# megvii-research/OccDepth

Measured on AMD Instinct MI355X. Metric: frames/sec forward, SemanticKITTI stereo->256x256x32 voxels, higher is better.
Workload: dtype f32 storage and accumulate; matrix arithmetic as 3x bf16 split (hi + mid + lo of both operands, six v_mfma_f32_32x32x16_bf16 per K step; error vs float64 tested within 1.5x of the exact-fp32 kernels', measured 0.8-1.1x) in the head convolutions (K2s3), the small-volume 3x3x3 convolutions and transpo

## Files before the change

### occdepth_amd/csrc/conv3d_bf16.hip

```cpp
#include "device.h"

#include <algorithm>
#include <cstddef>
#include <cstdlib>
#include <cstring>

using occd::FastDiv;

namespace {

struct PhaseBP {
    const u32x4* wpk;
    int KX, KY, KZ, oox, ooy, ooz, YIN, ZIN;
    FastDiv div_zin;
};
constexpr int kMaxPhasesB = 8;

struct ConvBP {
    const void* in;
    const float* bias;
    const void* res1;
    const void* res2;
    void* out;
    int X, Y, Z, cin8, cin16, in_cs, in_coff;
    int K16tot, NTtot;
    int out_cs, out_coff, res1_cs, res1_coff, res2_cs, res2_coff;
    int SX, SY, SZ, DX, DY, DZ, PX, PY, PZ;
    int Xo, Yo, Zo, OX, OY, OZ, osx, osy, osz;
    int act_in, act_out, cout_store;
    int TY, TZ, ytiles, ztiles, nwg;
    int nph_log2;
    int ph_fast;
    FastDiv div_tz, div_ztiles, div_ytiles;
    PhaseBP ph[kMaxPhasesB];
};

__device__ __forceinline__ f32x4 unpack_lo(u32x2 v) {
    f32x4 r;
    r.x = __builtin_bit_cast(float, v.x << 16);
    r.y = __builtin_bit_cast(float, v.x & 0xffff0000u);
    r.z = __builtin_bit_cast(float, v.y << 16);
    r.w = __builtin_bit_cast(float, v.y & 0xffff0000u);
    return r;
}

constexpr int kRSB = 80;
constexpr int kRSB3 = 208;


template <int MT, int NT, int WM, int WN, bool IN_BF16, bool OUT_BF16, int SPLIT = 1, int KS = 1>
__global__ void __launch_bounds__(WM* WN * KS * 64) conv3d_bf16_kernel(const ConvBP p) {
    constexpr int NTH = WM * WN * 64;
    constexpr int RSB = SPLIT == 3 ? kRSB3 : kRSB;
    static_assert(SPLIT == 1 || (SPLIT == 3 && !IN_BF16 && !OUT_BF16), "the 3-way split takes and returns float32");
    extern __shared__ __attribute__((aligned(16))) unsigned char slab_all[];

    const int lane = threadIdx.x & 63;
    const int wave_all = __builtin_amdgcn_readfirstlane(threadIdx.x >> 6);
    const int kg = KS == 1 ? 0 : wave_all / (WM * WN);
    const int wave = wave_all - kg * (WM * WN);
    const int tid = threadIdx.x - kg * NTH;
    const int wm = wave / WN;
    const int wn = wave - wm * WN;
    const int li = lane & 31;
    const int h = lane >> 5;

    uint32_t bid = xcd_remap(blockIdx.x, p.nwg);
    const uint32_t ph_mask = (1u << p.nph_log2) - 1u;
    const uint32_t ph_i = p.ph_fast ? bid & ph_mask : blockIdx.y & ph_mask;
    if (p.ph_fast) bid >>= p.nph_log2;
    const uint32_t t1 = occd_fastdiv(bid, p.div_ztiles);
    const int zt = bid - t1 * p.ztiles;
    const uint32_t t2 = occd_fastdiv(t1, p.div_ytiles);
    const int yt = t1 - t2 * p.ytiles;
    const int xo = t2;
    const int b = p.ph_fast ? blockIdx.y : blockIdx.y >> p.nph_log2;
    const PhaseBP& ph = p.ph[ph_i];
// ... 16 lines not shown

    f32x16 acc[MT][NT];
#pragma unroll
    for (int mt = 0; mt < MT; ++mt)
#pragma unroll
        for (int nt = 0; nt < NT; ++nt)
#pragma unroll
            for (int r = 0; r < 16; ++r) acc[mt][nt][r] = 0.f;

    const int y_in0 = yt * p.TY * p.SY - p.PY;
    const int z_in0 = zt * p.TZ * p.SZ - p.PZ;
    const size_t w_step = (size_t)p.NTtot * 64;
    const size_t w_img = (size_t)ph.KX * ph.KY * ph.KZ * p.K16tot * w_step;
    const u32x4* const wlane = ph.wpk + lane;
    const int rows = ph.YIN * ph.ZIN;
    unsigned char* const slab = slab_all + (size_t)kg * rows * RSB;
    const int n_chunks = (p.cin16 + 31) / 32;
    const int chunk_iters = (n_chunks + KS - 1) / KS;

#define OCCD_MFMA1(WS, XS)                                                                                          \
    _Pragma("unroll") for (int nt = 0; nt < NT; ++nt) _Pragma("unroll") for (int mt = 0; mt < MT; ++mt) acc[mt][nt] = \
        __builtin_amdgcn_mfma_f32_32x32x16_bf16(__builtin_bit_cast(bf16x8, b_cur[nt][WS]),                         \
                                                __builtin_bit_cast(bf16x8, a_cur[mt][XS]), acc[mt][nt], 0, 0, 0)
#define OCCD_MFMA_BLOCK()                                                  \
    if (SPLIT == 3) {                                                      \
        OCCD_MFMA1(SPLIT == 3 ? 1 : 0, SPLIT == 3 ? 1 : 0);                \
        OCCD_MFMA1(0, SPLIT == 3 ? 2 : 0);                                 \
        OCCD_MFMA1(SPLIT == 3 ? 2 : 0, 0);                                 \
        OCCD_MFMA1(0, SPLIT == 3 ? 1 : 0);                                 \
        OCCD_MFMA1(SPLIT == 3 ? 1 : 0, 0);                                 \
    }                                                                      \
    OCCD_MFMA1(0, 0)

    for (int kx = 0; kx < ph.KX; ++kx) {
        const int xi = xo * p.SX - p.PX + kx * p.DX;
        if (xi < 0 || xi >= p.X) continue;
        const size_t plane = ((size_t)(b * p.X + xi) * p.Y) * p.Z * p.in_cs + p.in_coff;
        for (int ci = 0; ci < chunk_iters; ++ci) {
            const int c0 = (ci * KS + kg) * 32;
            const bool active = KS == 1 || c0 < p.cin16;
            const int ck = active ? min(32, p.cin16 - c0) : 16;
            const int k16n = ck >> 4;
            const int sh = k16n;
            const int S = active ? ph.KY * ph.KZ * k16n : 0;
            const u32x4* wp = wlane + ((size_t)(kx * ph.KY * ph.KZ) * p.K16tot + (active ? c0 >> 4 : 0)) * w_step;

            u32x4 b_cur[NT][SPLIT];
#pragma unroll
            for (int nt = 0; nt < NT; ++nt)
#pragma unroll
                for (int sp = 0; sp < SPLIT; ++sp) b_cur[nt][sp] = wp[wofs[nt] + sp * w_img];

            __syncthreads();
            const int F = rows << sh;
            for (int f0 = 0; active && f0 < F; f0 += NTH * 4) {
                u32x4 v[4][SPLIT];
                int dst[4];
#pragma unroll
                for (int u = 0; u < 4; ++u) {
                    const int f = f0 + u * NTH + tid;
                    const int fc = min(f, F - 1);
                    const uint32_t row = (uint32_t)fc >> sh;
                    const int c8 = fc & ((1 << sh) - 1);
                    const uint32_t yi = occd_fastdiv(row, ph.div_zin);
                    const int zi = (int)row - (int)yi * ph.ZIN;
                    const int y = y_in0 + (int)yi, z = z_in0 + zi;
                    const int c = c0 + c8 * 8;
                    const bool ok = f < F && c < p.cin8 && (unsigned)y < (unsigned)p.Y && (unsigned)z < (unsigned)p.Z;
                    const int yc = min(max(y, 0), p.Y - 1), zc = min(max(z, 0), p.Z - 1);
                    const int cc = min(c, p.cin8 - 8);
                    const size_t e = plane + ((size_t)yc * p.Z + zc) * p.in_cs + cc;
                    u32x4 w[SPLIT];
                    if (IN_BF16) {
                        w[0] = *(const u32x4*)((const uint16_t*)p.in + e);
                        if (p.act_in == OCCD_ACT_RELU) {
#pragma unroll
                            for (int q = 0; q < 4; ++q) {
                                uint32_t d = w[0][q];
                                if (d & 0x80000000u) d &= 0x0000ffffu;
                                if (d & 0x00008000u) d &= 0xffff0000u;
                                w[0][q] = d;
                            }
                        }
                    } else {
                        f32x4 lo = *(const f32x4*)((const float*)p.in + e);
                        f32x4 hi = *(const f32x4*)((const float*)p.in + e + 4);
                        if (p.act_in == OCCD_ACT_RELU) { lo = act3d_x4(lo, OCCD_ACT_RELU); hi = act3d_x4(hi, OCCD_ACT_RELU); }
                        else if (SPLIT == 3 && p.act_in == OCCD_ACT_SIGMOID) {
                            lo = act3d_x4(lo, OCCD_ACT_SIGMOID); hi = act3d_x4(hi, OCCD_ACT_SIGMOID);
                        }
                        if (SPLIT == 3) split3_bf16x8(lo, hi, w[0], w[SPLIT == 3 ? 1 : 0], w[SPLIT == 3 ? 2 : 0]);
                        else w[0] = pack_bf16x8(lo, hi);
                    }
#pragma unroll
                    for (int sp = 0; sp < SPLIT; ++sp) v[u][sp] = ok ? w[sp] : u32x4{0u, 0u, 0u, 0u};
                    dst[u] = f < F ? (int)row * RSB + c8 * 16 : -1;
                }
#pragma unroll
                for (int u = 0; u < 4; ++u)
                    if (dst[u] >= 0) {
#pragma unroll
                        for (int sp = 0; sp < SPLIT; ++sp) *(u32x4*)(slab + dst[u] + sp * 64) = v[u][sp];
                    }
            }
            __syncthreads();

            int ky = 0, kz = 0, kl = 0;
            int lds_off = 0;
            u32x4 a_cur[MT][SPLIT];
#pragma unroll
            for (int mt = 0; mt < MT; ++mt)
#pragma unroll
                for (int sp = 0; sp < SPLIT; ++sp) a_cur[mt][sp] = *(const u32x4*)(slab + rowbase[mt] + sp * 64);

            for (int s = 0; s < S - 1; ++s) {
                ++kl;
                lds_off += 32;
                wp += w_step;
                if (kl == k16n) {
                    kl = 0;
                    wp += (size_t)(p.K16tot - k16n) * w_step;
                    if (++kz == ph.KZ) { kz = 0; ++ky; }
                    lds_off = (ky * p.DY * ph.ZIN + kz * p.DZ) * RSB;
                }
                u32x4 a_nxt[MT][SPLIT], b_nxt[NT][SPLIT];
#pragma unroll
                for (int mt = 0; mt < MT; ++mt)
#pragma unroll
                    for (int sp = 0; sp < SPLIT; ++sp) a_nxt[mt][sp] = *(const u32x4*)(slab + rowbase[mt] + lds_off + sp * 64);
#pragma unroll
                for (int nt = 0; nt < NT; ++nt)
#pragma unroll
                    for (int sp = 0; sp < SPLIT; ++sp) b_nxt[nt][sp] = wp[wofs[nt] + sp * w_img];
                OCCD_MFMA_BLOCK();
#pragma unroll
                for (int mt = 0; mt < MT; ++mt)
#pragma unroll
                    for (int sp = 0; sp < SPLIT; ++sp) a_cur[mt][sp] = a_nxt[mt][sp];
#pragma unroll
                for (int nt = 0; nt < NT; ++nt)
#pragma unroll
                    for (int sp = 0; sp < SPLIT; ++sp) b_cur[nt][sp] = b_nxt[nt][sp];
            }
            if (active) { OCCD_MFMA_BLOCK(); }
        }
    }
#undef OCCD_MFMA1
#undef OCCD_MFMA_BLOCK

    if (KS > 1) {
        float* red = reinterpret_cast<float*>(slab_all);
        __syncthreads();
        if (kg > 0) {
#pragma unroll
            for (int mt = 0; mt < MT; ++mt)
#pragma unroll
                for (int nt = 0; nt < NT; ++nt)
#pragma unroll
                    for (int r = 0; r < 16; ++r)
                        red[((((kg - 1) * WM * WN + wave) * MT + mt) * NT + nt) * 1024 + r * 64 + lane] = acc[mt][nt][r];
        }
        __syncthreads();
        if (kg > 0) return;
#pragma unroll
        for (int g = 1; g < KS; ++g)
#pragma unroll
            for (int mt = 0; mt < MT; ++mt)
#pragma unroll
                for (int nt = 0; nt < NT; ++nt)
#pragma unroll
                    for (int r = 0; r < 16; ++r)
                        acc[mt][nt][r] += red[((((g - 1) * WM * WN + wave) * MT + mt) * NT + nt) * 1024 + r * 64 + lane];
    }

#pragma unroll
    for (int mt = 0; mt < MT; ++mt) {
        const uint32_t m = (wm * MT + mt) * 32 + li;
        const uint32_t yl = occd_fastdiv(m, p.div_tz);
        const uint32_t zl = m - yl * p.TZ;
        const int yo = yt * p.TY + (int)yl, zo = zt * p.TZ + (int)zl;
        const bool ok = yl < (uint32_t)p.TY && yo < p.Yo && zo < p.Zo;
        const size_t vox = ((size_t)(b * p.OX + xo * p.osx + ph.oox) * p.OY + (yo * p.osy + ph.ooy)) * p.OZ +
                           (zo * p.osz + ph.ooz);
#pragma unroll
        for (int nt = 0; nt < NT; ++nt) {
#pragma unroll
            for (int g = 0; g < 4; ++g) {
                const int c = (nt0 + nt) * 32 + 8 * g + 4 * h;
                if (ok && c < p.cout_store) {
                    f32x4 v = {acc[mt][nt][4 * g], acc[mt][nt][4 * g + 1], acc[mt][nt][4 * g + 2],
                               acc[mt][nt][4 * g + 3]};
                    if (p.bias != nullptr) v += *(const f32x4*)(p.bias + c);
                    if (p.act_out == OCCD_ACT_RELU_PRE) v = act3d_x4(v, OCCD_ACT_RELU);
                    if (OUT_BF16) {
                        if (p.res1 != nullptr)
                            v += unpack_lo(*(const u32x2*)((const uint16_t*)p.res1 + vox * p.res1_cs + p.res1_coff + c));
                        if (p.res2 != nullptr)
                            v += unpack_lo(*(const u32x2*)((const uint16_t*)p.res2 + vox * p.res2_cs + p.res2_coff + c));
                    } else {
                        if (p.res1 != nullptr) v += *(const f32x4*)((const float*)p.res1 + vox * p.res1_cs + p.res1_coff + c);
                        if (p.res2 != nullptr) v += *(const f32x4*)((const float*)p.res2 + vox * p.res2_cs + p.res2_coff + c);
                    }
                    if (p.act_out == OCCD_ACT_RELU) v = act3d_x4(v, OCCD_ACT_RELU);
                    if (OUT_BF16) {
                        bf16x4 o = {(__bf16)v.x, (__bf16)v.y, (__bf16)v.z, (__bf16)v.w};
                        *(u32x2*)((uint16_t*)p.out + vox * p.out_cs + p.out_coff + c) = __builtin_bit_cast(u32x2, o);
                    } else {
                        *(f32x4*)((float*)p.out + vox * p.out_cs + p.out_coff + c) = v;
                    }
                }
            }
        }
    }
}
// ... 58 lines not shown
    const int lane = (i >> 3) & 63;
    long t = i >> 9;
    const int nt = t % NT; t /= NT;
    const int k16 = t % K16; t /= K16;
    const int tap = (int)t;
    const int co = nt * 32 + (lane & 31);
    const int ci = k16 * 16 + (lane >> 5) * 8 + j;
    float v = 0.f;
    if (co < cout && ci < cin) {
        if (layout == 0) v = w[((size_t)co * cin + ci) * taps + tap];
        else if (layout == 1) v = w[((size_t)ci * cout + co) * taps + tap];
        else v = w[(size_t)ci * cout + co];
        if (scale != nullptr) v *= scale[co];
        v *= 0.5f / fac[co];
    }
    const _Float16 hi = (_Float16)v;
    wpk[i] = __builtin_bit_cast(uint16_t, hi);
    wpk[i + total] = __builtin_bit_cast(uint16_t, (_Float16)((float)hi * (1.f / 2048.f)));
    wpk[i + 2 * total] = __builtin_bit_cast(uint16_t, (_Float16)(v - (float)hi));
}

struct VariantB {
    int MT, NT, WM, WN, KS;
    void (*kern[3])(const ConvBP);
};

#define OCCD_VARIANT_B(MT, NT, WM, WN) \
    VariantB { MT, NT, WM, WN, 1, { conv3d_bf16_kernel<MT, NT, WM, WN, false, false>, conv3d_bf16_kernel<MT, NT, WM, WN, true, true>, nullptr } }
#define OCCD_VARIANT_B3(MT, NT, WM, WN) \
    VariantB { MT, NT, WM, WN, 1, { conv3d_bf16_kernel<MT, NT, WM, WN, false, false>, conv3d_bf16_kernel<MT, NT, WM, WN, true, true>, \
                                    conv3d_bf16_kernel<MT, NT, WM, WN, false, false, 3> } }

const VariantB kVariantsB[] = {
    OCCD_VARIANT_B(4, 1, 4, 1),
    OCCD_VARIANT_B3(2, 1, 4, 1),
    OCCD_VARIANT_B3(1, 1, 4, 1),
    OCCD_VARIANT_B(4, 2, 4, 1),
    OCCD_VARIANT_B3(2, 2, 4, 1),
    OCCD_VARIANT_B(4, 2, 2, 2),
    OCCD_VARIANT_B3(2, 2, 2, 2),
    OCCD_VARIANT_B3(1, 2, 2, 2),
    VariantB { 1, 1, 1, 4, 4, { nullptr, nullptr, conv3d_bf16_kernel<1, 1, 1, 4, false, false, 3, 4> } },
};
constexpr int kNumVariantsB = sizeof(kVariantsB) / sizeof(kVariantsB[0]);
constexpr size_t kMaxLdsB = 160 * 1024;

struct TilingB {
    int TY, TZ, YIN, ZIN, ytiles, ztiles, ngroups;
    size_t lds;
    long nwg;
    double cost;
};

bool plan_b(const occd_conv3d_args* a, const VariantB& v, int NTtot, TilingB* best, int rsb) {
    const int mwg = v.MT * v.WM * 32;
    bool found = false;
    int cands[16];
    int nc = 0;
    if (a->Zo <= mwg) cands[nc++] = a->Zo;
    for (int tz = 8; tz <= mwg; tz *= 2)
        if (tz < a->Zo) cands[nc++] = tz;
    for (int i = 0; i < nc; ++i) {
        TilingB t;
        t.TZ = cands[i];
        t.TY = mwg / t.TZ;
// ... 92 lines not shown
    return pack_bf16_gather(w, scale, wpk, cout, cin, ntaps, s_co, s_ci, tap_ofs, 3, stream);
}

static int pack_bf16_gather(const float* w, const float* scale, void* wpk, int32_t cout, int32_t cin, int32_t ntaps,
                            int64_t s_co, int64_t s_ci, const int32_t* tap_ofs, int nsplit, void* stream) {
    if (!w || !wpk || !tap_ofs || ntaps <= 0 || ntaps > occd::kMaxTaps) return OCCD_EINVAL;
    const int64_t total = occd_packed_weight_bf16_elems(cout, cin, ntaps);
    if (total <= 0) return OCCD_EINVAL;
    occd::TapMap tm{};
    tm.s_co = s_co; tm.s_ci = s_ci;
    for (int i = 0; i < ntaps; ++i) tm.ofs[i] = tap_ofs[i];
    const int K16 = (cin + 15) / 16, NT = (cout + 31) / 32;
    const int th = 256;
    const long blocks = (total + th - 1) / th;
    occd::ProfScope prof("pack_weights_bf16", (hipStream_t)stream, 0.0, (double)total * 6);
    hipLaunchKernelGGL(pack_weights_bf16_kernel, dim3((unsigned)blocks), dim3(th), 0, (hipStream_t)stream, w, scale,
                       (uint16_t*)wpk, cout, cin, ntaps, K16, NT, 3, (long)total, nsplit, tm);
    return occd::check_launch();
}

namespace {

int validate_b(const occd_conv3d_args* a, int32_t dtype) {
    if (!a || !a->in || !a->wpk || !a->out || dtype < 0 || dtype > 3) return OCCD_EINVAL;
    const int ksel = dtype;
    if (dtype >= 2) dtype = 0;
    if (a->batch <= 0 || a->X <= 0 || a->Y <= 0 || a->Z <= 0 || a->cin <= 0 || a->cout <= 0) return OCCD_EINVAL;
    if (a->kx <= 0 || a->ky <= 0 || a->kz <= 0 || a->sx <= 0 || a->sy <= 0 || a->sz <= 0) return OCCD_EINVAL;
    if (a->Xo <= 0 || a->Yo <= 0 || a->Zo <= 0) return OCCD_EINVAL;
    const int cin8 = (a->cin + 7) & ~7;
    const int cin16 = (a->cin + 15) & ~15;
    const int NTtot = (a->cout + 31) / 32;
    const int al = dtype == 1 ? 7 : 3;
    const int esz = dtype == 1 ? 2 : 4;
    if ((a->in_cs & al) || (a->in_coff & al) || a->in_coff + cin8 > a->in_cs) return OCCD_EINVAL;
    if ((reinterpret_cast<uintptr_t>(a->in) & 15) || (reinterpret_cast<uintptr_t>(a->wpk) & 15)) return OCCD_EINVAL;
    if (a->cout_store < a->cout || a->cout_store > NTtot * 32 || a->out_coff + a->cout_store > a->out_cs)
        return OCCD_EINVAL;
    if ((a->cout_store & 3) || (a->out_cs & 3) || (a->out_coff & 3) ||
        (reinterpret_cast<uintptr_t>(a->out) & (4 * esz - 1)))
        return OCCD_EINVAL;
    if (a->res1 && ((a->res1_cs & 3) || (a->res1_coff & 3) || (reinterpret_cast<uintptr_t>(a->res1) & (4 * esz - 1)) ||
                    a->res1_coff + a->cout_store > a->res1_cs))
        return OCCD_EINVAL;
    if (a->res2 && ((a->res2_cs & 3) || (a->res2_coff & 3) || (reinterpret_cast<uintptr_t>(a->res2) & (4 * esz - 1)) ||
                    a->res2_coff + a->cout_store > a->res2_cs))
        return OCCD_EINVAL;
    if (a->bias && (reinterpret_cast<uintptr_t>(a->bias) & 15)) return OCCD_EINVAL;
    if ((a->Xo - 1) * a->o_stride_x + a->o_off_x >= a->OX || (a->Yo - 1) * a->o_stride_y + a->o_off_y >= a->OY ||
        (a->Zo - 1) * a->o_stride_z + a->o_off_z >= a->OZ)
        return OCCD_EINVAL;
    if (a->act_in != OCCD_ACT_NONE && a->act_in != OCCD_ACT_RELU && !(a->act_in == OCCD_ACT_SIGMOID && ksel == 2)) return OCCD_EINVAL;
    if (a->act_out != OCCD_ACT_NONE && a->act_out != OCCD_ACT_RELU && a->act_out != OCCD_ACT_RELU_PRE)
        return OCCD_EINVAL;
    return OCCD_OK;
}

int launch_b(const occd_conv3d_args* a, int n, int32_t dtype, hipStream_t stream) {
    const int ksel = dtype;
    if (dtype == 2) dtype = 0;
    const int esz = dtype == 1 ? 2 : 4;
    const int cin8 = (a->cin + 7) & ~7;
    const int cin16 = (a->cin + 15) & ~15;
    const int NTtot = (a->cout + 31) / 32;
    occd_conv3d_args big = a[0];
    for (int i = 1; i < n; ++i) {
        big.ky = a[i].ky > big.ky ? a[i].ky : big.ky;
        big.kz = a[i].kz > big.kz ? a[i].kz : big.kz;
    }
    const long copies = (long)a->batch * n;
    int order[kNumVariantsB];
    int no = 0;
    if (a->tile_hint > 0 && a->tile_hint <= kNumVariantsB) {
        order[no++] = a->tile_hint - 1;
    } else if (NTtot == 1) {
        order[no++] = 0; order[no++] = 1; order[no++] = 2;
    } else if (NTtot == 2) {
        order[no++] = 3; order[no++] = 4; order[no++] = 6; order[no++] = 7;
    } else {
        order[no++] = 5; order[no++] = 6; order[no++] = 7;
    }
    const int rsb = ksel == 2 ? kRSB3 : kRSB;
    int pick = -1;
    TilingB til{};
    for (int i = 0; i < no; ++i) {
        TilingB t{};
        if (kVariantsB[order[i]].kern[ksel] == nullptr) continue;
        if (!plan_b(&big, kVariantsB[order[i]], NTtot, &t, rsb)) continue;
        pick = order[i];
        til = t;
        if (t.nwg * t.ngroups * copies >= 512) break;
    }
    if (pick < 0) return OCCD_ENOMEM;
    if (ksel == 2 && a->tile_hint == 0 && til.nwg * til.ngroups * copies <= 320 && cin16 >= 128 && NTtot % 4 == 0) {
        TilingB t{};
        if (plan_b(&big, kVariantsB[8], NTtot, &t, rsb) && t.nwg * t.ngroups * copies <= 1024) {
            pick = 8;
            til = t;
        }
    }
    const VariantB& v = kVariantsB[pick];

    ConvBP p{};
    p.in = a->in; p.bias = a->bias; p.res1 = a->res1; p.res2 = a->res2; p.out = a->out;
    p.X = a->X; p.Y = a->Y; p.Z = a->Z; p.cin8 = cin8; p.cin16 = cin16; p.in_cs = a->in_cs; p.in_coff = a->in_coff;
    p.K16tot = cin16 / 16; p.NTtot = NTtot;
    p.out_cs = a->out_cs; p.out_coff = a->out_coff;
    p.res1_cs = a->res1_cs; p.res1_coff = a->res1_coff; p.res2_cs = a->res2_cs; p.res2_coff = a->res2_coff;
    p.SX = a->sx; p.SY = a->sy; p.SZ = a->sz;
    p.DX = a->dx; p.DY = a->dy; p.DZ = a->dz; p.PX = a->px; p.PY = a->py; p.PZ = a->pz;
    p.Xo = a->Xo; p.Yo = a->Yo; p.Zo = a->Zo; p.OX = a->OX; p.OY = a->OY; p.OZ = a->OZ;
    p.osx = a->o_stride_x; p.osy = a->o_stride_y; p.osz = a->o_stride_z;
    p.act_in = a->act_in; p.act_out = a->act_out; p.cout_store = a->cout_store;
    p.TY = til.TY; p.TZ = til.TZ;
    p.ytiles = til.ytiles; p.ztiles = til.ztiles; p.nwg = (int)til.nwg;
    p.div_tz = occd::make_fastdiv(til.TZ);
    p.div_ztiles = occd::make_fastdiv(til.ztiles); p.div_ytiles = occd::make_fastdiv(til.ytiles);
    p.nph_log2 = n == 1 ? 0 : n == 2 ? 1 : n == 4 ? 2 : 3;
    static const bool phase_fast = occd::env_flag("OCCD_PHASE_FAST", false);
    p.ph_fast = n > 1 && phase_fast ? 1 : 0;
    if (p.ph_fast) p.nwg = (int)(til.nwg * n);
    if (til.nwg * n >= (1L << 24)) return OCCD_EINVAL;
    int ord[kMaxPhasesB];
    for (int i = 0; i < n; ++i) ord[i] = i;
    std::stable_sort(ord, ord + n, [&](int l, int r) { return a[l].kx * a[l].ky * a[l].kz > a[r].kx * a[r].ky * a[r].kz; });
    double flops = 0.0, bytes = 0.0;
    const double pos = (double)a->batch * a->Xo * a->Yo * a->Zo;
    for (int i = 0; i < n; ++i) {
        const occd_conv3d_args* ai = a + ord[i];
        PhaseBP& ph = p.ph[i];
        ph.wpk = (const u32x4*)ai->wpk;
        ph.KX = ai->kx; ph.KY = ai->ky; ph.KZ = ai->kz;
        ph.oox = ai->o_off_x; ph.ooy = ai->o_off_y; ph.ooz = ai->o_off_z;
        ph.YIN = (til.TY - 1) * ai->sy + (ai->ky - 1) * ai->dy + 1;
        ph.ZIN = (til.TZ - 1) * ai->sz + (ai->kz - 1) * ai->dz + 1;
        ph.div_zin = occd::make_fastdiv(ph.ZIN);
        if ((size_t)ph.YIN * ph.ZIN * rsb * v.KS > til.lds) return OCCD_EINVAL;
        const double taps = (double)ai->kx * ai->ky * ai->kz;
        flops += 2.0 * pos * taps * ai->cin * ai->cout;
        bytes += (double)esz * ((i == 0 ? (double)a->batch * a->X * a->Y * a->Z * a->cin : 0.0) +
                                pos * a->cout * (1 + (a->res1 != nullptr) + (a->res2 != nullptr))) + 2.0 * taps * a->cin * a->cout;
    }
    if (copies > 65535) return OCCD_EINVAL;

    void (*kern)(const ConvBP) = v.kern[ksel];
    if (til.lds > 64 * 1024 && occd::ensure_big_lds(reinterpret_cast<const void*>(kern)) != OCCD_OK) return OCCD_ELAUNCH;
    occd::ProfScope prof(n > 1 ? "conv3d_bf16x3_phases" : ksel == 2 ? "conv3d_bf16x3" : dtype == 1 ? "conv3d_bf16s" : "conv3d_bf16",
                         stream, flops, bytes);
    hipLaunchKernelGGL(kern, p.ph_fast ? dim3((unsigned)(til.nwg * n), (unsigned)a->batch, (unsigned)til.ngroups)
                                       : dim3((unsigned)til.nwg, (unsigned)copies, (unsigned)til.ngroups),
                       dim3(v.WM * v.WN * v.KS * 64), til.lds, stream, p);
    return occd::check_launch();
}

}

extern "C" int occd_conv3d_bf16_fwd(const occd_conv3d_args* a, int32_t dtype, void* stream) {
    const int bad = validate_b(a, dtype);
    if (bad != OCCD_OK) return bad;
    if (dtype == 3) {
        const int r = occd::try_conv3d_c32_slide_x3(a, (hipStream_t)stream, true);
        return r < 0 ? r : r == 0 ? OCCD_EINVAL : OCCD_OK;
    }
    if (dtype == 2) {
        const int r = occd::try_conv3d_c32_slide_x3(a, (hipStream_t)stream);
        if (r != 0) return r < 0 ? r : OCCD_OK;
    }
    return launch_b(a, 1, dtype, (hipStream_t)stream);
}

// ... 13 lines not shown
```

### occdepth_amd/fused.py

```python
import os

import torch

from . import hip
from .hip import ACT_NONE, ACT_RELU, ACT_RELU_PRE, ACT_SIGMOID, Vox


_warned_eval_with_grad = False


def needs_autograd(module):
    if module.training:
        return True
    if torch.is_grad_enabled():
        global _warned_eval_with_grad
        if not _warned_eval_with_grad:
            _warned_eval_with_grad = True
            import warnings
            warnings.warn("occdepth_amd: eval-mode forward with autograd enabled runs the differentiable ATen path; "
                          "wrap inference in torch.no_grad() to take the HIP eval path", stacklevel=3)
        return True
    return False


# ... 95 lines not shown
BF16X3 = _parse_bf16x3(os.environ.get("OCCDEPTH_BF16X3", "head"))


def set_bf16x3(on):
    global BF16X3
    BF16X3 = "all" if on is True else _parse_bf16x3(str(on)) if on else False


def _parse_head_split(v):
    v = (v or "f16x2").strip().lower()
    if v not in ("f16x2", "bf16x3"):
        raise ValueError(f"OCCDEPTH_HEAD_SPLIT={v!r}: expected f16x2 or bf16x3")
    return v


HEAD_SPLIT = _parse_head_split(os.environ.get("OCCDEPTH_HEAD_SPLIT", "f16x2"))


def set_head_split(v):
    global HEAD_SPLIT
    HEAD_SPLIT = _parse_head_split(v)


class _DualW:

    def __init__(self, f32, x3, f16x2=None):
        self.f32, self.x3, self.f16x2 = f32, x3, f16x2


BF16X3_DILATED = os.environ.get("OCCDEPTH_BF16X3_DILATED", "0") == "1"


def _head_weight(w, layout):
    return layout == 0 and w.dim() == 5 and tuple(w.shape[2:]) == (3, 3, 3) and w.shape[0] <= 32 and 24 < w.shape[1] <= 32


BF16X3_SMALLVOL = os.environ.get("OCCDEPTH_BF16X3_SMALLVOL", "1") == "1"
SMALLVOL_MAX_VOXELS = 8192
SMALLVOL_KERNELS = ((3, 3, 3), (1, 1, 1)) if os.environ.get("OCCDEPTH_BF16X3_SMALLVOL_K1", "0") == "1" else ((3, 3, 3),)


def _smallvol_weight(w, layout):
    if not BF16X3_SMALLVOL:
        return False
    if layout == 2:
        return (1, 1, 1) in SMALLVOL_KERNELS and w.dim() == 2 and w.shape[0] >= 128 and w.shape[0] % 16 == 0 and w.shape[1] % 128 == 0
    return (layout == 0 and w.dim() == 5 and tuple(w.shape[2:]) in SMALLVOL_KERNELS and w.shape[1] >= 128
            and w.shape[1] % 16 == 0 and w.shape[0] % 128 == 0)


def _f16x2_ok(w, scale):
    if not w.is_cuda:
        return False
    ws = w if scale is None else w * scale.view(-1, *([1] * (w.dim() - 1)))
    return bool(torch.isfinite(ws).all())


def _pack_w(w, scale=None, layout=0):
    if BF16X3 == "all" or (BF16X3 == "head" and (_head_weight(w, layout) or _smallvol_weight(w, layout))):
        f16 = (hip.pack_weights_f16x2(w, scale, layout)
               if HEAD_SPLIT == "f16x2" and _head_weight(w, layout) and _f16x2_ok(w, scale) else None)
        return _DualW(hip.pack_weights(w, scale, layout), hip.pack_weights_bf16(w, scale, layout, split3=True), f16)
    return hip.pack_weights(w, scale, layout)


def _smallvol_eligible(x, wpk, cout, kernel, out, **kw):
    if not BF16X3_SMALLVOL or tuple(kernel) not in SMALLVOL_KERNELS or kw.get("cin") not in (None, x.C) or x.C < 128 or cout % 128:
        return False
    if x.cs % 8 or x.coff % 8 or x.buf.dtype != torch.float32:
        return False
    pos = kw.get("out_pos")
    if pos is None:
        st, dl, pd = kw.get("stride", (1, 1, 1)), kw.get("dilation", (1, 1, 1)), kw.get("padding", (0, 0, 0))
        pos = tuple((n + 2 * p - d * (k - 1) - 1) // s + 1 for n, p, d, s, k in zip(x.dims, pd, dl, st, kernel))
    return x.batch * pos[0] * pos[1] * pos[2] <= SMALLVOL_MAX_VOXELS and kw.get("tile_hint", 0) == 0


def _conv3d(x, wpk, bias, cout, kernel, out, **kw):
    if isinstance(wpk, _DualW):
        if hip.c32x3_eligible(x, cout, kernel, out, **kw):
            if wpk.f16x2 is not None:
                return hip.conv3d_f16x2(x, wpk.f16x2, bias, cout, kernel, out, **kw)
            return hip.conv3d_bf16(x, wpk.x3, bias, cout, kernel, out, split3=True, **kw)
        if _smallvol_eligible(x, wpk, cout, kernel, out, **kw):
            return hip.conv3d_bf16(x, wpk.x3, bias, cout, kernel, out, split3=True, **kw)
        aligned = x.cs % 8 == 0 and x.coff % 8 == 0
        dil = tuple(kw.get("dilation", (1, 1, 1)))
        big = kernel[0] * kernel[1] * kernel[2] >= 8
        if BF16X3 == "all" and aligned and big and (dil == (1, 1, 1) or BF16X3_DILATED) and kw.get("cin") is None and \
                kw.get("act_in", ACT_NONE) in (ACT_NONE, ACT_RELU):
            return hip.conv3d_bf16(x, wpk.x3, bias, cout, kernel, out, split3=True, **kw)
        wpk = wpk.f32
    return hip.conv3d(x, wpk, bias, cout, kernel, out, **kw)


class ConvPlan:

    def __init__(self, conv, bn=None, pool=None):
        self.conv, self.bn = conv, bn
        self.pool = _triple(pool) if pool is not None else None
        self._key = None
        self._wpk = self._bias = None

    @property
    def cout(self):
        return self.conv.out_channels

    def _prepare(self):
        key = (_stamp(self.conv, self.bn), BF16X3, HEAD_SPLIT)
        if key == self._key:
            return
        w = self.conv.weight.detach().float()
        dev = w.device
        cout = self.cout
        scale, shift = _bn_affine(self.bn, cout, dev)
        if self.conv.bias is not None:
            cb = self.conv.bias.detach().float()
            shift = shift + (cb * scale if scale is not None else cb)
        if self.pool is not None:
            kx, ky, kz = self.pool
            w = (w / float(kx * ky * kz)).expand(-1, -1, kx, ky, kz).contiguous()
        self._wpk = _pack_w(w, scale)
        self._bias = _pad_bias(shift, cout)
        self._wrows = None
        if self.pool is None and tuple(w.shape[2:]) == (1, 1, 1) and _triple(self.conv.stride) == (1, 1, 1):
            w2 = w.reshape(cout, -1)
            if ROWS_GEMM and w2.is_cuda and w2.shape[1] % 16 == 0 and cout % 8 == 0:
                self._wrows = hip.RowsGemmWeights((w2 * scale.view(-1, 1) if scale is not None else w2).t().contiguous())
        self._key = key

    def geometry(self):
        if self.pool is not None:
# ... 7 lines not shown

    def __call__(self, x, out=None, res1=None, res2=None, act_in=ACT_NONE, act_out=ACT_NONE):
        self._prepare()
        k, s, d, p = self.geometry()
        if out is None:
            out = Vox.empty(x.batch, self.out_dims(x.dims), self.cout, x.buf.device)
        if (ROWS_GEMM and self._wrows is not None and res2 is None and x.buf.is_cuda and _rows_gemm_wins(x, self._wrows.K)
                and hip.rows_gemm_supported(self._wrows.K, self.cout, x, out, res1)):
            return hip.rows_gemm(x, self._wrows, out, bias=self._bias, res=res1, act_in=act_in, act_out=act_out)
        return _conv3d(x, self._wpk, self._bias, self.cout, k, out, stride=s, dilation=d, padding=p,
                          res1=res1, res2=res2, act_in=act_in, act_out=act_out)


class DerivedConvPlan:

    def __init__(self, modules, derive, padding=(1, 1, 1), dilation=(1, 1, 1), stride=(1, 1, 1)):
        self.modules, self.derive = list(modules), derive
        self.padding, self.dilation, self.stride = padding, dilation, stride
        self._key = None
        self._wpk = self._bias = None
        self.cout = self.kernel = None

    def _prepare(self):
        key = (_stamp(*self.modules), BF16X3, HEAD_SPLIT)
        if key == self._key:
            return
        w, b = self.derive()
        w = w.detach().float().contiguous()
        self.cout, self.kernel = w.shape[0], tuple(w.shape[2:])
        self._wpk = _pack_w(w)
        self._bias = _pad_bias(b.detach().float(), self.cout) if b is not None else None
        self._key = key

    def __call__(self, x, out=None, res1=None, res2=None, act_in=ACT_NONE, act_out=ACT_NONE, out_cs=None):
        self._prepare()
        if out is None:
            dims = tuple((n + 2 * p - d * (k - 1) - 1) // s + 1
                         for n, k, s, d, p in zip(x.dims, self.kernel, self.stride, self.dilation, self.padding))
            out = Vox.empty(x.batch, dims, self.cout, x.buf.device, cs=out_cs)
        return _conv3d(x, self._wpk, self._bias, self.cout, self.kernel, out, stride=self.stride,
                          dilation=self.dilation, padding=self.padding, res1=res1, res2=res2, act_in=act_in,
                          act_out=act_out)


PHASES_ONE_LAUNCH = os.environ.get("OCCDEPTH_PHASES_ONE_LAUNCH", "1") == "1"
PHASES_X3 = os.environ.get("OCCDEPTH_PHASES_X3", "1") == "1"

# ... 1 lines not shown
class ConvTransposePlan:

    def __init__(self, convt, bn=None):
        self.convt, self.bn = convt, bn
        ks, st = _triple(convt.kernel_size), _triple(convt.stride)
        pd, op = _triple(convt.padding), _triple(convt.output_padding)
        if ks != (3, 3, 3) or pd != (1, 1, 1) or _triple(convt.dilation) != (1, 1, 1):
            raise NotImplementedError("only the k3/p1 transposed convolutions of OccDepth are planned")
        if st == (2, 2, 2) and op == (1, 1, 1):
            self.up = 2
        elif st == (1, 1, 1) and op == (0, 0, 0):
            self.up = 1
        else:
            raise NotImplementedError(f"ConvTranspose3d stride {st} output_padding {op}")
        self._key = None
        self._phases = None
        self._bias = None

    @property
    def cout(self):
        return self.convt.out_channels

    def _prepare(self):
        key = (_stamp(self.convt, self.bn), BF16X3, PHASES_X3)
        if key == self._key:
            return
        x3 = bool(BF16X3) and PHASES_X3 and PHASES_ONE_LAUNCH

        def pack(w, scale):
            if x3:
                return _DualW(hip.pack_weights(w, scale), hip.pack_weights_bf16(w, scale, split3=True))
            return _pack_w(w, scale)
        wt = self.convt.weight.detach().float()
        dev = wt.device
        scale, shift = _bn_affine(self.bn, self.cout, dev)
        if self.convt.bias is not None:
            cb = self.convt.bias.detach().float()
            shift = shift + (cb * scale if scale is not None else cb)
        w = wt.permute(1, 0, 2, 3, 4)
        phases = []
        if self.up == 1:
            phases.append(((0, 0, 0), (3, 3, 3), (1, 1, 1), _pack_w(w.flip(2, 3, 4).contiguous(), scale)))
        else:
            taps = ([1], [2, 0])
            for px in (0, 1):
                for py in (0, 1):
                    for pz in (0, 1):
                        sub = w[:, :, taps[px]][:, :, :, taps[py]][:, :, :, :, taps[pz]].contiguous()
                        phases.append(((px, py, pz), tuple(sub.shape[2:]), (0, 0, 0), pack(sub, scale)))
        self._phases = phases
        self._bias = _pad_bias(shift, self.cout)
        self._key = key

    def out_dims(self, dims):
        return tuple(n * self.up for n in dims)

    def __call__(self, x, out=None, res1=None, act_out=ACT_NONE):
        self._prepare()
        if out is None:
            out = Vox.empty(x.batch, self.out_dims(x.dims), self.cout, x.buf.device)
        def phase(off, kern, pad, wpk):
            return lambda: _conv3d(x, wpk, self._bias, self.cout, kern, out, padding=pad, res1=res1, act_out=act_out,
                                   out_pos=x.dims, o_stride=(self.up,) * 3, o_off=off)

        if PHASES_ONE_LAUNCH and len(self._phases) > 1 and BF16X3 and PHASES_X3 and x.buf.dtype == torch.float32 and \
                x.cs % 8 == 0 and x.coff % 8 == 0 and all(isinstance(ph[3], _DualW) for ph in self._phases):
            return hip.conv3d_phases(x, [(wpk.x3, kern, off) for off, kern, _, wpk in self._phases], self._bias, self.cout, out,
                                     res1=res1, act_out=act_out, out_pos=x.dims, o_stride=(self.up,) * 3, split3=True)
        if PHASES_ONE_LAUNCH and len(self._phases) > 1 and BF16X3 != "all":
            return hip.conv3d_phases(x, [(wpk.f32 if isinstance(wpk, _DualW) else wpk, kern, off) for off, kern, _, wpk in self._phases],
                                     self._bias, self.cout, out, res1=res1, act_out=act_out, out_pos=x.dims,
                                     o_stride=(self.up,) * 3)
        thunks = [phase(*ph) for ph in self._phases]
        if x.buf.is_cuda and len(thunks) > 1:
            run_parallel(thunks)
        else:
            for th in thunks:
                th()
        return out


ROWS_GEMM = os.environ.get("OCCDEPTH_ROWS_GEMM", "0") == "1"


def _rows_gemm_wins(x, K):
    rows = x.batch * x.dims[0] * x.dims[1] * x.dims[2]
    return rows <= 65536 or K >= 256


# ... 54 lines not shown
```

### occdepth_amd/hip.py

```python
import ctypes
import os
from ctypes import c_int32, c_int64, c_void_p

import torch

from . import abi

_HERE = os.path.dirname(os.path.abspath(__file__))
LIB_PATH = os.path.join(_HERE, "libocc_hip.so")

EXPORTS = abi.EXPORTS
ABI_VERSION = abi.ABI_VERSION
MAX_VIEWS = abi.CONSTANTS["OCCD_MAX_VIEWS"]
MAX_SCALES = abi.CONSTANTS["OCCD_MAX_SCALES"]
ACT_NONE = abi.CONSTANTS["OCCD_ACT_NONE"]
ACT_RELU = abi.CONSTANTS["OCCD_ACT_RELU"]
ACT_SIGMOID = abi.CONSTANTS["OCCD_ACT_SIGMOID"]
ACT_RELU_PRE = abi.CONSTANTS["OCCD_ACT_RELU_PRE"]
OPTIM_CHUNK = abi.CONSTANTS["OCCD_OPTIM_CHUNK"]
MAX_REGIONS = abi.CONSTANTS["OCCD_MAX_REGIONS"]

Conv3dArgs = abi.STRUCTS["occd_conv3d_args"]
WgradArgs = abi.STRUCTS["occd_conv3d_wgrad_args"]
FlospArgs = abi.STRUCTS["occd_flosp_args"]
# ... 185 lines not shown
        out_pos = tuple((n + 2 * p - d * (k - 1) - 1) // s + 1
                        for n, p, d, k, s in zip(x.dims, padding, dilation, kernel, stride))
    a.Xo, a.Yo, a.Zo = out_pos
    a.o_stride_x, a.o_stride_y, a.o_stride_z = o_stride
    a.o_off_x, a.o_off_y, a.o_off_z = o_off
    a.act_in, a.act_out = act_in, act_out
    a.cout_store = min(round_up(cout, 8), out.cs - out.coff, round_up(cout, 32))
    a.tile_hint = tile_hint
    if _PROFILING:
        set_tag("%d>%d k%d%d%d s%d%d%d d%d%d%d @%dx%dx%d" % ((a.cin, a.cout) + tuple(kernel) + tuple(stride)
                                                              + tuple(dilation) + tuple(x.dims)))
    return a


def conv3d(x, wpk, bias, cout, kernel, out, stride=(1, 1, 1), dilation=(1, 1, 1), padding=(0, 0, 0),
           res1=None, res2=None, act_in=ACT_NONE, act_out=ACT_NONE, out_pos=None, o_stride=(1, 1, 1),
           o_off=(0, 0, 0), cin=None, tile_hint=0):
    a = _conv3d_args(x, _f32(wpk, "wpk"), bias, cout, kernel, out, stride, dilation, padding, res1, res2, act_in, act_out,
                     out_pos, o_stride, o_off, cin, tile_hint, _f32)
    _check(load().occd_conv3d_fwd(ctypes.byref(a), _stream()), "occd_conv3d_fwd")
    return out


def conv3d_phases(x, phases, bias, cout, out, res1=None, act_out=ACT_NONE, out_pos=None, o_stride=(1, 1, 1), split3=False):
    n = len(phases)
    arr = (Conv3dArgs * n)()
    for i, (wpk, kernel, o_off) in enumerate(phases):
        a = _conv3d_args(x, _ptr(wpk, "wpk") if split3 else _f32(wpk, "wpk"), bias, cout, kernel, out, (1, 1, 1), (1, 1, 1),
                         (0, 0, 0), res1, None, ACT_NONE, act_out, out_pos, o_stride, o_off, None, 0, _f32)
        ctypes.memmove(ctypes.byref(arr, i * ctypes.sizeof(Conv3dArgs)), ctypes.byref(a), ctypes.sizeof(Conv3dArgs))
    if _PROFILING:
        set_tag("%d>%d k333 s222 transposed: %d phases @%dx%dx%d" % ((x.C, cout, n) + tuple(x.dims)))
    if split3:
        _check(load().occd_conv3d_bf16_fwd_phases(arr, n, 2, _stream()), "occd_conv3d_bf16_fwd_phases")
    else:
        _check(load().occd_conv3d_fwd_phases(arr, n, _stream()), "occd_conv3d_fwd_phases")
    return out


def _act_ptr(dtype):
    def ptr(t, name):
        if t.dtype != dtype:
            raise RuntimeError(f"{name} must be {dtype} like the other activation tensors of the launch, got {t.dtype}")
        return _ptr(t, name)
    return ptr


def _storage_code(dtype):
    if dtype == torch.float32:
        return 0
    if dtype == torch.bfloat16:
        return 1
    raise RuntimeError(f"the bf16-MFMA kernels take float32 or bfloat16 activations, got {dtype}")


def pack_weights_bf16(w, scale=None, layout=0, split3=False):
    if layout == 2:
# ... 27 lines not shown
        raise RuntimeError("occd_packed_weight_f16x2_bytes: bad shape")
    out = torch.empty(n, device=w.device, dtype=torch.uint8)
    sc = scale.detach().float().contiguous() if scale is not None else None
    _check(load().occd_pack_weights_f16x2(_f32(w, "w"), _f32(sc, "scale") if sc is not None else None, _ptr(out, "wpk"),
                                          cout, cin, k[0], k[1], k[2], layout, _stream()), "occd_pack_weights_f16x2")
    return out


def conv3d_f16x2(x, wpk, bias, cout, kernel, out, **kw):
    if wpk.dtype != torch.uint8:
        raise RuntimeError("conv3d_f16x2 needs the image of pack_weights_f16x2")
    if x.buf.dtype != torch.float32:
        raise RuntimeError("the fp16 split takes float32 tensors")
    a = _conv3d_args(x, _ptr(wpk, "wpk"), bias, cout, kernel, out, kw.get("stride", (1, 1, 1)), kw.get("dilation", (1, 1, 1)),
                     kw.get("padding", (0, 0, 0)), kw.get("res1"), kw.get("res2"), kw.get("act_in", ACT_NONE),
                     kw.get("act_out", ACT_NONE), kw.get("out_pos"), kw.get("o_stride", (1, 1, 1)), kw.get("o_off", (0, 0, 0)),
                     kw.get("cin"), kw.get("tile_hint", 0), _act_ptr(x.buf.dtype))
    _check(load().occd_conv3d_bf16_fwd(ctypes.byref(a), 3, _stream()), "occd_conv3d_bf16_fwd (f16x2)")
    return out


def conv3d_bf16(x, wpk, bias, cout, kernel, out, stride=(1, 1, 1), dilation=(1, 1, 1), padding=(0, 0, 0),
                res1=None, res2=None, act_in=ACT_NONE, act_out=ACT_NONE, out_pos=None, o_stride=(1, 1, 1),
                o_off=(0, 0, 0), cin=None, tile_hint=0, split3=False):
    if wpk.dtype != torch.bfloat16:
        raise RuntimeError("conv3d_bf16 needs the bf16 weight image of pack_weights_bf16")
    if split3 and x.buf.dtype != torch.float32:
        raise RuntimeError("the 3-way split takes float32 tensors")
    ptr = _act_ptr(x.buf.dtype)
    a = _conv3d_args(x, _ptr(wpk, "wpk"), bias, cout, kernel, out, stride, dilation, padding, res1, res2, act_in, act_out,
                     out_pos, o_stride, o_off, cin, tile_hint, ptr)
    _check(load().occd_conv3d_bf16_fwd(ctypes.byref(a), 2 if split3 else _storage_code(x.buf.dtype), _stream()),
           "occd_conv3d_bf16_fwd")
    return out


GEMM_ACT = {None: abi.CONSTANTS["OCCD_GEMM_ACT_NONE"], "none": abi.CONSTANTS["OCCD_GEMM_ACT_NONE"],
            "swish": abi.CONSTANTS["OCCD_GEMM_ACT_SWISH"], "leaky": abi.CONSTANTS["OCCD_GEMM_ACT_LEAKY"]}


class GemmPacked:

    def __init__(self, w, role):
        if role not in ("a", "b") or w.dim() not in (2, 3) or w.dtype != torch.float32 or not w.is_cuda:
            raise RuntimeError("GemmPacked: a 2-D / 3-D float32 GPU tensor and role 'a' or 'b'")
        w = w.detach().contiguous()
        self.role, self.batch = role, (w.shape[0] if w.dim() == 3 else None)
# ... 1770 lines not shown
```

Before: 62.79.

## Use fp16 two-way split for small-volume 3x3x3 and transposed-phase convolutions

Adds a SPLIT==2 variant of the bf16 conv kernel that splits activations and weights into fp16 hi/lo pairs with a per-channel scale factor. It issues three f16 MFMAs per K step instead of six bf16 ones and uses a smaller LDS row stride. The default path now sends small-volume 3x3x3 convolutions and the transposed-conv phase launches through this kernel. That roughly halves matrix work in those layers, at the cost of fp16 range and accuracy risk, which is limited by the _f16x2_ok check and the weight scaling.

```diff
diff --git a/occdepth_amd/csrc/conv3d_bf16.hip b/occdepth_amd/csrc/conv3d_bf16.hip
--- a/occdepth_amd/csrc/conv3d_bf16.hip
+++ b/occdepth_amd/csrc/conv3d_bf16.hip
@@ -11,6 +11,7 @@
 
 struct PhaseBP {
     const u32x4* wpk;
+    const float* fac;
     int KX, KY, KZ, oox, ooy, ooz, YIN, ZIN;
     FastDiv div_zin;
 };
@@ -46,13 +47,15 @@
 
 constexpr int kRSB = 80;
 constexpr int kRSB3 = 208;
+constexpr int kRSB2 = 144;
 
 
 template <int MT, int NT, int WM, int WN, bool IN_BF16, bool OUT_BF16, int SPLIT = 1, int KS = 1>
 __global__ void __launch_bounds__(WM* WN * KS * 64) conv3d_bf16_kernel(const ConvBP p) {
     constexpr int NTH = WM * WN * 64;
-    constexpr int RSB = SPLIT == 3 ? kRSB3 : kRSB;
-    static_assert(SPLIT == 1 || (SPLIT == 3 && !IN_BF16 && !OUT_BF16), "the 3-way split takes and returns float32");
+    constexpr int RSB = SPLIT == 3 ? kRSB3 : SPLIT == 2 ? kRSB2 : kRSB;
+    constexpr int WIMG = SPLIT == 2 ? 2 : 1;
+    static_assert(SPLIT == 1 || ((SPLIT == 2 || SPLIT == 3) && !IN_BF16 && !OUT_BF16), "the splits take and return float32");
     extern __shared__ __attribute__((aligned(16))) unsigned char slab_all[];
 
     const int lane = threadIdx.x & 63;
@@ -115,15 +118,25 @@
     _Pragma("unroll") for (int nt = 0; nt < NT; ++nt) _Pragma("unroll") for (int mt = 0; mt < MT; ++mt) acc[mt][nt] = \
         __builtin_amdgcn_mfma_f32_32x32x16_bf16(__builtin_bit_cast(bf16x8, b_cur[nt][WS]),                         \
                                                 __builtin_bit_cast(bf16x8, a_cur[mt][XS]), acc[mt][nt], 0, 0, 0)
+#define OCCD_MFMA1H(W, XS)                                                                                          \
+    _Pragma("unroll") for (int nt = 0; nt < NT; ++nt) _Pragma("unroll") for (int mt = 0; mt < MT; ++mt) acc[mt][nt] = \
+        __builtin_amdgcn_mfma_f32_32x32x16_f16(W, __builtin_bit_cast(f16x8, a_cur[mt][XS]), acc[mt][nt], 0, 0, 0)
 #define OCCD_MFMA_BLOCK()                                                  \
-    if (SPLIT == 3) {                                                      \
+    if (SPLIT == 2) {                                                      \
+        f16x8 w_hs[NT];                                                    \
+        _Pragma("unroll") for (int nt = 0; nt < NT; ++nt)                  \
+            w_hs[nt] = __builtin_bit_cast(f16x8, b_cur[nt][0]) * (_Float16)(1.f / 2048.f); \
+        OCCD_MFMA1H(__builtin_bit_cast(f16x8, b_cur[nt][SPLIT == 2 ? 1 : 0]), 0); \
+        OCCD_MFMA1H(w_hs[nt], SPLIT == 2 ? 1 : 0);                         \
+        OCCD_MFMA1H(__builtin_bit_cast(f16x8, b_cur[nt][0]), 0);           \
+    } else if (SPLIT == 3) {                                               \
         OCCD_MFMA1(SPLIT == 3 ? 1 : 0, SPLIT == 3 ? 1 : 0);                \
         OCCD_MFMA1(0, SPLIT == 3 ? 2 : 0);                                 \
         OCCD_MFMA1(SPLIT == 3 ? 2 : 0, 0);                                 \
         OCCD_MFMA1(0, SPLIT == 3 ? 1 : 0);                                 \
         OCCD_MFMA1(SPLIT == 3 ? 1 : 0, 0);                                 \
     }                                                                      \
-    OCCD_MFMA1(0, 0)
+    if (SPLIT != 2) { OCCD_MFMA1(0, 0); }
 
     for (int kx = 0; kx < ph.KX; ++kx) {
         const int xi = xo * p.SX - p.PX + kx * p.DX;
@@ -142,7 +155,7 @@
 #pragma unroll
             for (int nt = 0; nt < NT; ++nt)
 #pragma unroll
-                for (int sp = 0; sp < SPLIT; ++sp) b_cur[nt][sp] = wp[wofs[nt] + sp * w_img];
+                for (int sp = 0; sp < SPLIT; ++sp) b_cur[nt][sp] = wp[wofs[nt] + sp * WIMG * w_img];
 
             __syncthreads();
             const int F = rows << sh;
@@ -183,6 +196,7 @@
                             lo = act3d_x4(lo, OCCD_ACT_SIGMOID); hi = act3d_x4(hi, OCCD_ACT_SIGMOID);
                         }
                         if (SPLIT == 3) split3_bf16x8(lo, hi, w[0], w[SPLIT == 3 ? 1 : 0], w[SPLIT == 3 ? 2 : 0]);
+                        else if (SPLIT == 2) split2_f16x8(lo, hi, w[0], w[SPLIT == 2 ? 1 : 0]);
                         else w[0] = pack_bf16x8(lo, hi);
                     }
 #pragma unroll
@@ -224,7 +238,7 @@
 #pragma unroll
                 for (int nt = 0; nt < NT; ++nt)
 #pragma unroll
-                    for (int sp = 0; sp < SPLIT; ++sp) b_nxt[nt][sp] = wp[wofs[nt] + sp * w_img];
+                    for (int sp = 0; sp < SPLIT; ++sp) b_nxt[nt][sp] = wp[wofs[nt] + sp * WIMG * w_img];
                 OCCD_MFMA_BLOCK();
 #pragma unroll
                 for (int mt = 0; mt < MT; ++mt)
@@ -239,6 +253,7 @@
         }
     }
 #undef OCCD_MFMA1
+#undef OCCD_MFMA1H
 #undef OCCD_MFMA_BLOCK
 
     if (KS > 1) {
@@ -283,6 +298,7 @@
                 if (ok && c < p.cout_store) {
                     f32x4 v = {acc[mt][nt][4 * g], acc[mt][nt][4 * g + 1], acc[mt][nt][4 * g + 2],
                                acc[mt][nt][4 * g + 3]};
+                    if (SPLIT == 2) v *= *(const f32x4*)(ph.fac + c);
                     if (p.bias != nullptr) v += *(const f32x4*)(p.bias + c);
                     if (p.act_out == OCCD_ACT_RELU_PRE) v = act3d_x4(v, OCCD_ACT_RELU);
                     if (OUT_BF16) {
@@ -387,14 +403,14 @@
 
 struct VariantB {
     int MT, NT, WM, WN, KS;
-    void (*kern[3])(const ConvBP);
+    void (*kern[4])(const ConvBP);
 };
 
 #define OCCD_VARIANT_B(MT, NT, WM, WN) \
-    VariantB { MT, NT, WM, WN, 1, { conv3d_bf16_kernel<MT, NT, WM, WN, false, false>, conv3d_bf16_kernel<MT, NT, WM, WN, true, true>, nullptr } }
+    VariantB { MT, NT, WM, WN, 1, { conv3d_bf16_kernel<MT, NT, WM, WN, false, false>, conv3d_bf16_kernel<MT, NT, WM, WN, true, true>, nullptr, nullptr } }
 #define OCCD_VARIANT_B3(MT, NT, WM, WN) \
     VariantB { MT, NT, WM, WN, 1, { conv3d_bf16_kernel<MT, NT, WM, WN, false, false>, conv3d_bf16_kernel<MT, NT, WM, WN, true, true>, \
-                                    conv3d_bf16_kernel<MT, NT, WM, WN, false, false, 3> } }
+                                    conv3d_bf16_kernel<MT, NT, WM, WN, false, false, 3>, conv3d_bf16_kernel<MT, NT, WM, WN, false, false, 2> } }
 
 const VariantB kVariantsB[] = {
     OCCD_VARIANT_B(4, 1, 4, 1),
@@ -405,7 +421,8 @@
     OCCD_VARIANT_B(4, 2, 2, 2),
     OCCD_VARIANT_B3(2, 2, 2, 2),
     OCCD_VARIANT_B3(1, 2, 2, 2),
-    VariantB { 1, 1, 1, 4, 4, { nullptr, nullptr, conv3d_bf16_kernel<1, 1, 1, 4, false, false, 3, 4> } },
+    VariantB { 1, 1, 1, 4, 4, { nullptr, nullptr, conv3d_bf16_kernel<1, 1, 1, 4, false, false, 3, 4>,
+                                conv3d_bf16_kernel<1, 1, 1, 4, false, false, 2, 4> } },
 };
 constexpr int kNumVariantsB = sizeof(kVariantsB) / sizeof(kVariantsB[0]);
 constexpr size_t kMaxLdsB = 160 * 1024;
@@ -544,7 +561,7 @@
 namespace {
 
 int validate_b(const occd_conv3d_args* a, int32_t dtype) {
-    if (!a || !a->in || !a->wpk || !a->out || dtype < 0 || dtype > 3) return OCCD_EINVAL;
+    if (!a || !a->in || !a->wpk || !a->out || dtype < 0 || dtype > 4) return OCCD_EINVAL;
     const int ksel = dtype;
     if (dtype >= 2) dtype = 0;
     if (a->batch <= 0 || a->X <= 0 || a->Y <= 0 || a->Z <= 0 || a->cin <= 0 || a->cout <= 0) return OCCD_EINVAL;
@@ -579,8 +596,8 @@
 }
 
 int launch_b(const occd_conv3d_args* a, int n, int32_t dtype, hipStream_t stream) {
-    const int ksel = dtype;
-    if (dtype == 2) dtype = 0;
+    const int ksel = dtype == 4 ? 3 : dtype;
+    if (dtype >= 2) dtype = 0;
     const int esz = dtype == 1 ? 2 : 4;
     const int cin8 = (a->cin + 7) & ~7;
     const int cin16 = (a->cin + 15) & ~15;
@@ -602,7 +619,7 @@
     } else {
         order[no++] = 5; order[no++] = 6; order[no++] = 7;
     }
-    const int rsb = ksel == 2 ? kRSB3 : kRSB;
+    const int rsb = ksel == 2 ? kRSB3 : ksel == 3 ? kRSB2 : kRSB;
     int pick = -1;
     TilingB til{};
     for (int i = 0; i < no; ++i) {
@@ -614,7 +631,7 @@
         if (t.nwg * t.ngroups * copies >= 512) break;
     }
     if (pick < 0) return OCCD_ENOMEM;
-    if (ksel == 2 && a->tile_hint == 0 && til.nwg * til.ngroups * copies <= 320 && cin16 >= 128 && NTtot % 4 == 0) {
+    if (ksel >= 2 && a->tile_hint == 0 && til.nwg * til.ngroups * copies <= 320 && cin16 >= 128 && NTtot % 4 == 0) {
         TilingB t{};
         if (plan_b(&big, kVariantsB[8], NTtot, &t, rsb) && t.nwg * t.ngroups * copies <= 1024) {
             pick = 8;
@@ -652,6 +669,9 @@
         const occd_conv3d_args* ai = a + ord[i];
         PhaseBP& ph = p.ph[i];
         ph.wpk = (const u32x4*)ai->wpk;
+        ph.fac = ksel == 3 ? reinterpret_cast<const float*>(reinterpret_cast<const uint16_t*>(ai->wpk) +
+                                                            3 * (size_t)ai->kx * ai->ky * ai->kz * (cin16 / 16) * NTtot * 512)
+                           : nullptr;
         ph.KX = ai->kx; ph.KY = ai->ky; ph.KZ = ai->kz;
         ph.oox = ai->o_off_x; ph.ooy = ai->o_off_y; ph.ooz = ai->o_off_z;
         ph.YIN = (til.TY - 1) * ai->sy + (ai->ky - 1) * ai->dy + 1;
@@ -667,7 +687,8 @@
 
     void (*kern)(const ConvBP) = v.kern[ksel];
     if (til.lds > 64 * 1024 && occd::ensure_big_lds(reinterpret_cast<const void*>(kern)) != OCCD_OK) return OCCD_ELAUNCH;
-    occd::ProfScope prof(n > 1 ? "conv3d_bf16x3_phases" : ksel == 2 ? "conv3d_bf16x3" : dtype == 1 ? "conv3d_bf16s" : "conv3d_bf16",
+    occd::ProfScope prof(n > 1 ? (ksel == 3 ? "conv3d_bf16x3_phases_f16x2" : "conv3d_bf16x3_phases") :
+                         ksel == 3 ? "conv3d_bf16x3_f16x2" : ksel == 2 ? "conv3d_bf16x3" : dtype == 1 ? "conv3d_bf16s" : "conv3d_bf16",
                          stream, flops, bytes);
     hipLaunchKernelGGL(kern, p.ph_fast ? dim3((unsigned)(til.nwg * n), (unsigned)a->batch, (unsigned)til.ngroups)
                                        : dim3((unsigned)til.nwg, (unsigned)copies, (unsigned)til.ngroups),
diff --git a/occdepth_amd/fused.py b/occdepth_amd/fused.py
--- a/occdepth_amd/fused.py
+++ b/occdepth_amd/fused.py
@@ -141,10 +141,26 @@
     HEAD_SPLIT = _parse_head_split(v)
 
 
+def _parse_k2b_split(v):
+    v = (v or "f16x2").strip().lower()
+    if v not in ("f16x2", "bf16x3"):
+        raise ValueError(f"OCCDEPTH_K2B_SPLIT={v!r}: expected f16x2 or bf16x3")
+    return v
+
+
+K2B_SPLIT = _parse_k2b_split(os.environ.get("OCCDEPTH_K2B_SPLIT", "f16x2"))
+
+
+def set_k2b_split(v):
+    global K2B_SPLIT
+    K2B_SPLIT = _parse_k2b_split(v)
+
+
 class _DualW:
 
     def __init__(self, f32, x3, f16x2=None):
         self.f32, self.x3, self.f16x2 = f32, x3, f16x2
+        self.k2bh = False
 
 
 BF16X3_DILATED = os.environ.get("OCCDEPTH_BF16X3_DILATED", "0") == "1"
@@ -177,9 +193,13 @@
 
 def _pack_w(w, scale=None, layout=0):
     if BF16X3 == "all" or (BF16X3 == "head" and (_head_weight(w, layout) or _smallvol_weight(w, layout))):
-        f16 = (hip.pack_weights_f16x2(w, scale, layout)
-               if HEAD_SPLIT == "f16x2" and _head_weight(w, layout) and _f16x2_ok(w, scale) else None)
-        return _DualW(hip.pack_weights(w, scale, layout), hip.pack_weights_bf16(w, scale, layout, split3=True), f16)
+        head = HEAD_SPLIT == "f16x2" and _head_weight(w, layout)
+        k2bh = (not head and K2B_SPLIT == "f16x2" and layout == 0 and _smallvol_weight(w, 0)
+                and tuple(w.shape[2:]) == (3, 3, 3))
+        f16 = hip.pack_weights_f16x2(w, scale, layout) if (head or k2bh) and _f16x2_ok(w, scale) else None
+        dual = _DualW(hip.pack_weights(w, scale, layout), hip.pack_weights_bf16(w, scale, layout, split3=True), f16)
+        dual.k2bh = k2bh and f16 is not None
+        return dual
     return hip.pack_weights(w, scale, layout)
 
 
@@ -198,10 +218,12 @@
 def _conv3d(x, wpk, bias, cout, kernel, out, **kw):
     if isinstance(wpk, _DualW):
         if hip.c32x3_eligible(x, cout, kernel, out, **kw):
-            if wpk.f16x2 is not None:
+            if wpk.f16x2 is not None and not wpk.k2bh:
                 return hip.conv3d_f16x2(x, wpk.f16x2, bias, cout, kernel, out, **kw)
             return hip.conv3d_bf16(x, wpk.x3, bias, cout, kernel, out, split3=True, **kw)
         if _smallvol_eligible(x, wpk, cout, kernel, out, **kw):
+            if wpk.k2bh and tuple(kernel) == (3, 3, 3) and kw.get("act_in", ACT_NONE) in (ACT_NONE, ACT_RELU):
+                return hip.conv3d_bf16(x, wpk.f16x2, bias, cout, kernel, out, f16x2=True, **kw)
             return hip.conv3d_bf16(x, wpk.x3, bias, cout, kernel, out, split3=True, **kw)
         aligned = x.cs % 8 == 0 and x.coff % 8 == 0
         dil = tuple(kw.get("dilation", (1, 1, 1)))
@@ -226,7 +248,7 @@
         return self.conv.out_channels
 
     def _prepare(self):
-        key = (_stamp(self.conv, self.bn), BF16X3, HEAD_SPLIT)
+        key = (_stamp(self.conv, self.bn), BF16X3, HEAD_SPLIT, K2B_SPLIT)
         if key == self._key:
             return
         w = self.conv.weight.detach().float()
@@ -280,7 +302,7 @@
         self.cout = self.kernel = None
 
     def _prepare(self):
-        key = (_stamp(*self.modules), BF16X3, HEAD_SPLIT)
+        key = (_stamp(*self.modules), BF16X3, HEAD_SPLIT, K2B_SPLIT)
         if key == self._key:
             return
         w, b = self.derive()
@@ -328,14 +350,17 @@
         return self.convt.out_channels
 
     def _prepare(self):
-        key = (_stamp(self.convt, self.bn), BF16X3, PHASES_X3)
+        key = (_stamp(self.convt, self.bn), BF16X3, PHASES_X3, K2B_SPLIT)
         if key == self._key:
             return
         x3 = bool(BF16X3) and PHASES_X3 and PHASES_ONE_LAUNCH
 
         def pack(w, scale):
             if x3:
-                return _DualW(hip.pack_weights(w, scale), hip.pack_weights_bf16(w, scale, split3=True))
+                f16 = hip.pack_weights_f16x2(w, scale) if K2B_SPLIT == "f16x2" and _f16x2_ok(w, scale) else None
+                dual = _DualW(hip.pack_weights(w, scale), hip.pack_weights_bf16(w, scale, split3=True), f16)
+                dual.k2bh = f16 is not None
+                return dual
             return _pack_w(w, scale)
         wt = self.convt.weight.detach().float()
         dev = wt.device
@@ -371,6 +396,9 @@
 
         if PHASES_ONE_LAUNCH and len(self._phases) > 1 and BF16X3 and PHASES_X3 and x.buf.dtype == torch.float32 and \
                 x.cs % 8 == 0 and x.coff % 8 == 0 and all(isinstance(ph[3], _DualW) for ph in self._phases):
+            if all(ph[3].k2bh for ph in self._phases):
+                return hip.conv3d_phases(x, [(wpk.f16x2, kern, off) for off, kern, _, wpk in self._phases], self._bias, self.cout,
+                                         out, res1=res1, act_out=act_out, out_pos=x.dims, o_stride=(self.up,) * 3, f16x2=True)
             return hip.conv3d_phases(x, [(wpk.x3, kern, off) for off, kern, _, wpk in self._phases], self._bias, self.cout, out,
                                      res1=res1, act_out=act_out, out_pos=x.dims, o_stride=(self.up,) * 3, split3=True)
         if PHASES_ONE_LAUNCH and len(self._phases) > 1 and BF16X3 != "all":
diff --git a/occdepth_amd/hip.py b/occdepth_amd/hip.py
--- a/occdepth_amd/hip.py
+++ b/occdepth_amd/hip.py
@@ -231,8 +231,17 @@
     return out
 
 
-def conv3d_phases(x, phases, bias, cout, out, res1=None, act_out=ACT_NONE, out_pos=None, o_stride=(1, 1, 1), split3=False):
+def conv3d_phases(x, phases, bias, cout, out, res1=None, act_out=ACT_NONE, out_pos=None, o_stride=(1, 1, 1), split3=False,
+                  f16x2=False):
     n = len(phases)
+    if f16x2:
+        if split3:
+            raise RuntimeError("conv3d_phases: split3 and f16x2 are two forms of one launch, pick one")
+        if any(wpk.dtype != torch.uint8 for wpk, _, _ in phases):
+            raise RuntimeError("conv3d_phases(f16x2=True) needs the images of pack_weights_f16x2")
+        if x.buf.dtype != torch.float32:
+            raise RuntimeError("the fp16 split takes float32 tensors")
+        split3 = True
     arr = (Conv3dArgs * n)()
     for i, (wpk, kernel, o_off) in enumerate(phases):
         a = _conv3d_args(x, _ptr(wpk, "wpk") if split3 else _f32(wpk, "wpk"), bias, cout, kernel, out, (1, 1, 1), (1, 1, 1),
@@ -241,7 +250,7 @@
     if _PROFILING:
         set_tag("%d>%d k333 s222 transposed: %d phases @%dx%dx%d" % ((x.C, cout, n) + tuple(x.dims)))
     if split3:
-        _check(load().occd_conv3d_bf16_fwd_phases(arr, n, 2, _stream()), "occd_conv3d_bf16_fwd_phases")
+        _check(load().occd_conv3d_bf16_fwd_phases(arr, n, 4 if f16x2 else 2, _stream()), "occd_conv3d_bf16_fwd_phases")
     else:
         _check(load().occd_conv3d_fwd_phases(arr, n, _stream()), "occd_conv3d_fwd_phases")
     return out
@@ -315,7 +324,18 @@
 
 def conv3d_bf16(x, wpk, bias, cout, kernel, out, stride=(1, 1, 1), dilation=(1, 1, 1), padding=(0, 0, 0),
                 res1=None, res2=None, act_in=ACT_NONE, act_out=ACT_NONE, out_pos=None, o_stride=(1, 1, 1),
-                o_off=(0, 0, 0), cin=None, tile_hint=0, split3=False):
+                o_off=(0, 0, 0), cin=None, tile_hint=0, split3=False, f16x2=False):
+    if f16x2:
+        if split3:
+            raise RuntimeError("conv3d_bf16: split3 and f16x2 are two forms of one launch, pick one")
+        if wpk.dtype != torch.uint8:
+            raise RuntimeError("conv3d_bf16(f16x2=True) needs the image of pack_weights_f16x2")
+        if x.buf.dtype != torch.float32:
+            raise RuntimeError("the fp16 split takes float32 tensors")
+        a = _conv3d_args(x, _ptr(wpk, "wpk"), bias, cout, kernel, out, stride, dilation, padding, res1, res2, act_in, act_out,
+                         out_pos, o_stride, o_off, cin, tile_hint, _act_ptr(x.buf.dtype))
+        _check(load().occd_conv3d_bf16_fwd(ctypes.byref(a), 4, _stream()), "occd_conv3d_bf16_fwd (f16x2)")
+        return out
     if wpk.dtype != torch.bfloat16:
         raise RuntimeError("conv3d_bf16 needs the bf16 weight image of pack_weights_bf16")
     if split3 and x.buf.dtype != torch.float32:
```

Result: faster. 63.94, median of 6 (+1.8%).
